# latticeboltzmann/2d-lb

Measured on AMD Instinct MI355X. Metric: MLUPS (million lattice updates per second), fused D2Q9 BGK step, higher is better.
Workload: dtype f32

## Files before the change

### 2d-lb_amd/csrc/kernels_deep.h

```cpp
#pragma once

#ifdef LB_DIAG
#define LB_DEEP_NOCOLLIDE if (!(a.diag & 1))
#else
#define LB_DEEP_NOCOLLIDE
#endif

namespace {

constexpr int DEEP_RW = 1, DEEP_PFD = 1;
constexpr int DEEP_WSLOTS = 8;
constexpr bool deep_pairs(bool mask, int bc) { return !mask && bc == LB_BC_PERIODIC; }

template <int RW, int NL>
struct DeepState {
    Window w[RW > 0 ? RW : 1];
    f4a d0[NL];
    unsigned mhist;
};
typedef unsigned u4v __attribute__((ext_vector_type(4)));
struct DeepCtx {
    int lane, x4, ym, n_iter;
    bool store_lane;
    f4a (*mine)[64], (*other)[64];
    f4a (*ho)[64];
    f4a (*dma)[64];
    unsigned dma_off;
};
constexpr int DEEP_WHOLE = 0, DEEP_FRONT = 1, DEEP_BACK = 2;
constexpr int DEEP_HO_SLOTS = 10;

__device__ __forceinline__ void deep_window_load(f4a (*W)[64], int lane, int it, f4a d0, Window &w)
{
    const int gs = 2 + 3 * (it & 1);
    w.d0 = d0; w.d1 = W[0][lane]; w.d3 = W[1][lane];
    w.g2 = W[gs][lane]; w.g5 = W[gs + 1][lane]; w.g6 = W[gs + 2][lane];
}
template <bool DOWN>
__device__ __forceinline__ void deep_window_push(f4a (*W)[64], int lane, int it, f4a &d0, const f4a (&q)[9])
{
    typedef Dir<DOWN> D_;
    const int gs = 2 + 3 * (it & 1);
    d0 = q[0]; W[0][lane] = q[1]; W[1][lane] = q[3];
    W[gs][lane] = q[D_::A]; W[gs + 1][lane] = q[D_::B]; W[gs + 2][lane] = q[D_::C];
}
template <bool DOWN>
__device__ __forceinline__ void deep_publish(f4a (*W)[64], int lane, int gs, const f4a (&q)[9])
{
    typedef Dir<DOWN> D_;
    W[gs][lane] = q[D_::An]; W[gs + 1][lane] = q[D_::Bn]; W[gs + 2][lane] = q[D_::Cn];
}

constexpr int DEEP_NUM_RECORDS = -1;
__device__ __forceinline__ float *deep_uniform(const float *p)
{
    const unsigned long long v = (unsigned long long)p;
    const unsigned lo = __builtin_amdgcn_readfirstlane((unsigned)v), hi = __builtin_amdgcn_readfirstlane((unsigned)(v >> 32));
    return reinterpret_cast<float *>(((unsigned long long)hi << 32) | lo);
}
__device__ __forceinline__ f4a deep_buf_load(__amdgpu_buffer_rsrc_t r, int vo, int so, int imm)
{
    return __builtin_bit_cast(f4a, __builtin_amdgcn_raw_buffer_load_b128(r, vo + imm, so, 0));
}
template <int BC, bool MASK>
__device__ __forceinline__ void deep_row_load(const StepArgs &a, int r, int x4, Row1 &o)
{
    int ym, yp;
    o.have = step1_rows(a, r, o.rr, ym, yp);
    o.mk = uc4{0, 0, 0, 0};
    o.hsolid = false;
    o.hxc = -1;
    if (o.have) {
        const long long P = a.pitch, S = a.plane;
        const float *s = a.src;
        const int yl = o.rr;
        o.wp = WrapPatch{0.f, 0.f, 0.f, 0.f, 0.f, 0.f};
        if (BC == LB_BC_PERIODIC) {
            const int c = a.nx - 1 - x4;
            const bool wrap_w = x4 == 0, wrap_e = c >= 0 && c < 4;
            if (wrap_w) {
                o.wp.p1 = s[1 * S + (long long)yl * P + a.nx - 1];
                o.wp.p5 = s[5 * S + (long long)ym * P + a.nx - 1];
                o.wp.p8 = s[8 * S + (long long)yp * P + a.nx - 1];
            }
            if (wrap_e) {
                o.wp.w3 = s[3 * S + (long long)yl * P];
                o.wp.w6 = s[6 * S + (long long)ym * P];
                o.wp.w7 = s[7 * S + (long long)yp * P];
            }
        }
        const __amdgpu_buffer_rsrc_t r0 = __builtin_amdgcn_make_buffer_rsrc(deep_uniform(s + (long long)yl * P - 1), 0, DEEP_NUM_RECORDS, 0x00020000);
        const __amdgpu_buffer_rsrc_t rm = __builtin_amdgcn_make_buffer_rsrc(deep_uniform(s + (long long)ym * P - 1), 0, DEEP_NUM_RECORDS, 0x00020000);
        const __amdgpu_buffer_rsrc_t rp = __builtin_amdgcn_make_buffer_rsrc(deep_uniform(s + (long long)yp * P - 1), 0, DEEP_NUM_RECORDS, 0x00020000);
        const unsigned S4 = (unsigned)a.plane * 4u;
        const int vo = x4 * 4;
        o.q[0] = deep_buf_load(r0, vo, 0, 4);
        o.q[1] = deep_buf_load(r0, vo, (int)(S4), 0);
        o.q[2] = deep_buf_load(rm, vo, (int)(2u * S4), 4);
        o.q[3] = deep_buf_load(r0, vo, (int)(3u * S4), 8);
        o.q[4] = deep_buf_load(rp, vo, (int)(4u * S4), 4);
        o.q[5] = deep_buf_load(rm, vo, (int)(5u * S4), 0);
        o.q[6] = deep_buf_load(rm, vo, (int)(6u * S4), 8);
        o.q[7] = deep_buf_load(rp, vo, (int)(7u * S4), 8);
        o.q[8] = deep_buf_load(rp, vo, (int)(8u * S4), 0);
        if (MASK) o.mk = *reinterpret_cast<const uc4 *>(lane_ptr(a.mask + (long long)yl * a.fpitch, x4));
    } else {
        o.wp = WrapPatch{0.f, 0.f, 0.f, 0.f, 0.f, 0.f};
#pragma unroll
        for (int k = 0; k < 9; ++k) o.q[k] = f4a{0.f, 0.f, 0.f, 0.f};
    }
}
#ifdef LB_DIAG
constexpr bool DEEP_MANUAL = false;
#else
constexpr bool DEEP_MANUAL = true;
#endif
__device__ __forceinline__ u4v deep_rsrc_words(const float *p)
{
    const unsigned long long v = (unsigned long long)p;
    return u4v{(unsigned)__builtin_amdgcn_readfirstlane((unsigned)v), (unsigned)__builtin_amdgcn_readfirstlane((unsigned)(v >> 32)), (unsigned)DEEP_NUM_RECORDS,
               0x00020000u};
}
template <int BC, bool MASK>
__device__ __forceinline__ void deep_row_issue(const StepArgs &a, int r, int x4, Row1 &o)
{
    int ym, yp;
    o.have = step1_rows(a, r, o.rr, ym, yp);
    o.hsolid = false;
    o.hxc = -1;
    if (o.have) {
        const long long P = a.pitch, S = a.plane;
        const float *s = a.src;
        const int yl = o.rr;
        if (BC == LB_BC_PERIODIC) {
            const int c = a.nx - 1 - x4;
            const bool wrap_w = x4 == 0, wrap_e = c >= 0 && c < 4;
            if (wrap_w) {
                const float *e = s + a.nx - 1;
                asm volatile("global_load_dword a36, %0, off\n\tglobal_load_dword a37, %1, off\n\tglobal_load_dword a38, %2, off"
                             :: "v"(e + 1 * S + (long long)yl * P), "v"(e + 5 * S + (long long)ym * P), "v"(e + 8 * S + (long long)yp * P)
                             : "memory", "a36", "a37", "a38");
            }
            if (wrap_e) {
                asm volatile("global_load_dword a39, %0, off\n\tglobal_load_dword a40, %1, off\n\tglobal_load_dword a41, %2, off"
                             :: "v"(s + 3 * S + (long long)yl * P), "v"(s + 6 * S + (long long)ym * P), "v"(s + 7 * S + (long long)yp * P)
                             : "memory", "a39", "a40", "a41");
            }
        }
        const u4v r0 = deep_rsrc_words(s + (long long)yl * P - 1), rm = deep_rsrc_words(s + (long long)ym * P - 1),
                  rp = deep_rsrc_words(s + (long long)yp * P - 1);
        const unsigned S4 = (unsigned)a.plane * 4u;
        asm volatile("buffer_load_dwordx4 a[0:3], %0, %1, 0 offen offset:4\n\t"
                     "buffer_load_dwordx4 a[4:7], %0, %1, %4 offen\n\t"
                     "buffer_load_dwordx4 a[8:11], %0, %2, %5 offen offset:4\n\t"
                     "buffer_load_dwordx4 a[12:15], %0, %1, %6 offen offset:8\n\t"
                     "buffer_load_dwordx4 a[16:19], %0, %3, %7 offen offset:4\n\t"
                     "buffer_load_dwordx4 a[20:23], %0, %2, %8 offen\n\t"
                     "buffer_load_dwordx4 a[24:27], %0, %2, %9 offen offset:8\n\t"
                     "buffer_load_dwordx4 a[28:31], %0, %3, %10 offen offset:8\n\t"
                     "buffer_load_dwordx4 a[32:35], %0, %3, %11 offen"
                     :: "v"(x4 * 4), "s"(r0), "s"(rm), "s"(rp), "s"(S4), "s"(2u * S4), "s"(3u * S4), "s"(4u * S4), "s"(5u * S4), "s"(6u * S4),
                        "s"(7u * S4), "s"(8u * S4)
                     : "memory", "a0", "a1", "a2", "a3", "a4", "a5", "a6", "a7", "a8", "a9", "a10", "a11", "a12", "a13",
                       "a14", "a15", "a16", "a17", "a18", "a19", "a20", "a21", "a22", "a23", "a24", "a25", "a26", "a27", "a28",
                       "a29", "a30", "a31", "a32", "a33", "a34", "a35");
        if (MASK) asm volatile("global_load_dword a42, %0, off" :: "v"(lane_ptr(a.mask + (long long)yl * a.fpitch, x4)) : "memory", "a42");
    }
}
template <int BC, bool MASK, int N>
__device__ __forceinline__ void deep_row_take(Row1 &o)
{
    static_assert(N == 0 || N == 9 || N == 12, "the stores of one steady iteration, or nothing");
#define LB_DEEP_TAKE_OUTS "={a[0:3]}"(o.q[0]), "={a[4:7]}"(o.q[1]), "={a[8:11]}"(o.q[2]), "={a[12:15]}"(o.q[3]), \
                          "={a[16:19]}"(o.q[4]), "={a[20:23]}"(o.q[5]), "={a[24:27]}"(o.q[6]), "={a[28:31]}"(o.q[7]), "={a[32:35]}"(o.q[8])
    if (N == 0) asm volatile("s_waitcnt vmcnt(0)" : LB_DEEP_TAKE_OUTS :: "memory");
    else if (N == 9) asm volatile("s_waitcnt vmcnt(9)" : LB_DEEP_TAKE_OUTS :: "memory");
    else asm volatile("s_waitcnt vmcnt(12)" : LB_DEEP_TAKE_OUTS :: "memory");
#undef LB_DEEP_TAKE_OUTS
    o.wp = WrapPatch{0.f, 0.f, 0.f, 0.f, 0.f, 0.f};
    if (BC == LB_BC_PERIODIC)
        asm volatile("" : "={a36}"(o.wp.p1), "={a37}"(o.wp.p5), "={a38}"(o.wp.p8), "={a39}"(o.wp.w3), "={a40}"(o.wp.w6), "={a41}"(o.wp.w7));
    o.mk = uc4{0, 0, 0, 0};
    if (MASK) {
        unsigned m;
        asm volatile("" : "={a42}"(m));
        o.mk = __builtin_bit_cast(uc4, m);
    }
    if (!o.have) {
#pragma unroll
        for (int k = 0; k < 9; ++k) o.q[k] = f4a{0.f, 0.f, 0.f, 0.f};
        o.mk = uc4{0, 0, 0, 0};
    }
}

template <int BC, bool MASK>
__device__ __forceinline__ void deep_row_issue_lds(const StepArgs &a, int r, int x4, unsigned slot, Row1 &o)
{
    int ym, yp;
    o.have = step1_rows(a, r, o.rr, ym, yp);
    o.hsolid = false;
    o.hxc = -1;
    if (o.have) {
        const long long P = a.pitch, S = a.plane;
        const float *s = a.src;
        const int yl = o.rr;
        unsigned m0_kept;
        asm volatile("s_waitcnt lgkmcnt(0)" ::: "memory");
        if (BC == LB_BC_PERIODIC) {
            const int c = a.nx - 1 - x4;
            const bool wrap_w = x4 == 0, wrap_e = c >= 0 && c < 4;
            if (wrap_w) {
                const float *e = s + a.nx - 1;
                asm volatile("s_mov_b32 %0, m0\n\ts_mov_b32 m0, %4\n\ts_nop 0\n\tglobal_load_lds_dword %1, off\n\t"
                             "s_add_u32 m0, m0, 0x100\n\ts_nop 0\n\tglobal_load_lds_dword %2, off\n\t"
                             "s_add_u32 m0, m0, 0x100\n\ts_nop 0\n\tglobal_load_lds_dword %3, off\n\ts_mov_b32 m0, %0"
                             : "=&s"(m0_kept)
                             : "v"(e + 1 * S + (long long)yl * P), "v"(e + 5 * S + (long long)ym * P), "v"(e + 8 * S + (long long)yp * P),
                               "s"(slot + 9 * 1024 + 256)
                             : "memory", "scc");
            }
            if (wrap_e) {
                asm volatile("s_mov_b32 %0, m0\n\ts_mov_b32 m0, %4\n\ts_nop 0\n\tglobal_load_lds_dword %1, off\n\t"
                             "s_add_u32 m0, m0, 0x100\n\ts_nop 0\n\tglobal_load_lds_dword %2, off\n\t"
                             "s_add_u32 m0, m0, 0x100\n\ts_nop 0\n\tglobal_load_lds_dword %3, off\n\ts_mov_b32 m0, %0"
                             : "=&s"(m0_kept)
                             : "v"(s + 3 * S + (long long)yl * P), "v"(s + 6 * S + (long long)ym * P), "v"(s + 7 * S + (long long)yp * P),
                               "s"(slot + 9 * 1024 + 256)
                             : "memory", "scc");
            }
        }
        const u4v r0 = deep_rsrc_words(s + (long long)yl * P - 1), rm = deep_rsrc_words(s + (long long)ym * P - 1),
                  rp = deep_rsrc_words(s + (long long)yp * P - 1);
        const unsigned S4 = (unsigned)a.plane * 4u;
        const int v0 = x4 * 4, v4 = v0 + 4, v8 = v0 + 8;
        asm volatile("s_mov_b32 %0, m0\n\ts_mov_b32 m0, %15\n\ts_nop 0\n\tbuffer_load_dwordx4 %2, %4, 0 offen lds\n\t"
                     "s_add_u32 m0, m0, 0x400\n\ts_nop 0\n\tbuffer_load_dwordx4 %1, %4, %7 offen lds\n\t"
                     "s_add_u32 m0, m0, 0x400\n\ts_nop 0\n\tbuffer_load_dwordx4 %2, %5, %8 offen lds\n\t"
                     "s_add_u32 m0, m0, 0x400\n\ts_nop 0\n\tbuffer_load_dwordx4 %3, %4, %9 offen lds\n\t"
                     "s_add_u32 m0, m0, 0x400\n\ts_nop 0\n\tbuffer_load_dwordx4 %2, %6, %10 offen lds\n\t"
                     "s_add_u32 m0, m0, 0x400\n\ts_nop 0\n\tbuffer_load_dwordx4 %1, %5, %11 offen lds\n\t"
                     "s_add_u32 m0, m0, 0x400\n\ts_nop 0\n\tbuffer_load_dwordx4 %3, %5, %12 offen lds\n\t"
                     "s_add_u32 m0, m0, 0x400\n\ts_nop 0\n\tbuffer_load_dwordx4 %3, %6, %13 offen lds\n\t"
                     "s_add_u32 m0, m0, 0x400\n\ts_nop 0\n\tbuffer_load_dwordx4 %1, %6, %14 offen lds\n\ts_mov_b32 m0, %0"
                     : "=&s"(m0_kept)
                     : "v"(v0), "v"(v4), "v"(v8), "s"(r0), "s"(rm), "s"(rp), "s"(S4), "s"(2u * S4), "s"(3u * S4), "s"(4u * S4), "s"(5u * S4),
                       "s"(6u * S4), "s"(7u * S4), "s"(8u * S4), "s"(slot)
                     : "memory", "scc");
        if (MASK)
            asm volatile("s_mov_b32 %0, m0\n\ts_mov_b32 m0, %2\n\ts_nop 0\n\tglobal_load_lds_dword %1, off\n\ts_mov_b32 m0, %0"
                         : "=&s"(m0_kept) : "v"(lane_ptr(a.mask + (long long)yl * a.fpitch, x4)), "s"(slot + 9 * 1024) : "memory");
    }
}
template <int BC, bool MASK>
__device__ __forceinline__ void deep_row_take_lds(const f4a (*S)[64], int lane, Row1 &o)
{
    asm volatile("s_waitcnt vmcnt(0)" ::: "memory");
    if (o.have) {
#pragma unroll
        for (int k = 0; k < 9; ++k) o.q[k] = S[k][lane];
        const unsigned *X = reinterpret_cast<const unsigned *>(S[9]);
        o.mk = MASK ? __builtin_bit_cast(uc4, X[lane]) : uc4{0, 0, 0, 0};
        o.wp = WrapPatch{0.f, 0.f, 0.f, 0.f, 0.f, 0.f};
        if (BC == LB_BC_PERIODIC) {
            const float e1 = __builtin_bit_cast(float, X[64 + lane]), e2 = __builtin_bit_cast(float, X[128 + lane]),
                        e3 = __builtin_bit_cast(float, X[192 + lane]);
            o.wp = WrapPatch{e1, e2, e3, e1, e2, e3};
        }
    } else {
        o.wp = WrapPatch{0.f, 0.f, 0.f, 0.f, 0.f, 0.f};
#pragma unroll
        for (int k = 0; k < 9; ++k) o.q[k] = f4a{0.f, 0.f, 0.f, 0.f};
        o.mk = uc4{0, 0, 0, 0};
    }
}

__device__ __forceinline__ void deep_row_store(const StepArgs &a, int r, int x4, const f4a (&t)[9])
{
    const __amdgpu_buffer_rsrc_t rd = __builtin_amdgcn_make_buffer_rsrc(deep_uniform(a.dst + (long long)r * a.pitch), 0, DEEP_NUM_RECORDS, 0x00020000);
    const unsigned S4 = (unsigned)a.plane * 4u;
    const int vo = x4 * 4;
    asm volatile("" ::: "memory");
    if (a.nts != 0) {
#pragma unroll
        for (int k = 0; k < 9; ++k) __builtin_amdgcn_raw_buffer_store_b128(__builtin_bit_cast(u4v, t[k]), rd, vo, (int)(k * S4), 2);
    } else {
#pragma unroll
        for (int k = 0; k < 9; ++k) __builtin_amdgcn_raw_buffer_store_b128(__builtin_bit_cast(u4v, t[k]), rd, vo, (int)(k * S4), 0);
    }
}

template <int BC, bool MASK, bool MACRO, int D, int RW, bool DOWN, int NST, int S, int ROLE = DEEP_WHOLE>
__device__ __forceinline__ void deep_stage(const StepArgs &a, const DeepCtx &cx, const int i, const int it,
                                           DeepState<RW, D - 1 - RW> &st, f4a (&qin)[9], f4a &r4, f4a &u4, f4a &v4)
{
    if constexpr (S <= D) {
        constexpr int K = S - 1;
        const int lane = cx.lane, x4 = cx.x4;
        constexpr int L = K > RW ? K - RW - 1 : 0;
        f4a (*W)[64] = cx.mine + L * DEEP_WSLOTS;
        if constexpr (NST >= S) {
            int r, t0_, t1_;
            (void)step1_rows(a, DOWN ? cx.ym - 1 - (i - K) : cx.ym + (i - K), r, t0_, t1_);
            f4a t[9];
            if constexpr (K <= RW) {
                skirt_gather<DOWN>(st.w[K - 1], qin, t);
                window_push_dir<DOWN>(st.w[K - 1], qin);
            } else {
                Window w;
                deep_window_load(W, lane, it, st.d0[L], w);
                skirt_gather<DOWN>(w, qin, t);
                deep_window_push<DOWN>(W, lane, it, st.d0[L], qin);
            }
            LB_DEEP_NOCOLLIDE collide_row<BC, MASK, true>(a, x4, a.y0 + r, t, mask_bits(st.mhist, K), r4, u4, v4);
            if constexpr (S == D && ROLE == DEEP_FRONT) {
#pragma unroll
                for (int k = 0; k < 9; ++k) cx.ho[k][lane] = t[k];
                if (MASK) reinterpret_cast<unsigned *>(cx.ho[9])[lane] = __builtin_bit_cast(unsigned, mask_bits(st.mhist, K));
            } else if constexpr (S == D) {
#ifdef LB_DIAG
                if (!(a.diag & (1 << 22)))
#endif
                if (cx.store_lane) {
                    deep_row_store(a, r, x4, t);
                    if (MACRO) {
                        const long long m = (long long)r * a.fpitch;
                        store_moments(a, m, x4, r4, u4, v4);
                    }
                }
            } else {
                if constexpr (NST == S) {
                    if constexpr (S <= RW) deep_publish<DOWN>(cx.other + (D - 2 - RW) * DEEP_WSLOTS, lane, S == 1 ? 5 : 2, t);
                    else deep_publish<DOWN>(cx.other + (S - RW - 1) * DEEP_WSLOTS, lane, 2 + 3 * (S & 1), t);
                }
                deep_stage<BC, MASK, MACRO, D, RW, DOWN, NST, S + 1, ROLE>(a, cx, i, it, st, t, r4, u4, v4);
            }
        } else if constexpr (NST == S - 1) {
            if constexpr (K <= RW) window_push_dir<DOWN>(st.w[K - 1], qin);
            else deep_window_push<DOWN>(W, lane, it, st.d0[L], qin);
        }
    }
}

template <int BC, bool MASK, bool MACRO, int D, int RW, int PFD, bool DOWN, int NST, int PAR = -1, int ROLE = DEEP_WHOLE>
__device__ __forceinline__ void deep_iter(const StepArgs &a, const DeepCtx &cx, const int i_, DeepState<RW, D - 1 - RW> &st, Row1 &cur,
                                          Row1 &nxt)
{
    static_assert(RW >= 0 && RW <= 2 && D - 1 - RW >= 1 && (ROLE == DEEP_WHOLE ? D - 2 > RW : D - 2 >= RW),
                  "register windows hand over through the last LDS window while it is idle");
    static_assert((D - 1 - RW) * DEEP_WSLOTS <= 40, "a wave has 40 KB of LDS at four waves per CU");
    const int lane = cx.lane, x4 = cx.x4;
    const int i = NST < D ? NST - 1 : i_;
    const int it = PAR >= 0 ? PAR : i;
    auto row_at = [&](int p) { return DOWN ? cx.ym - 1 - p : cx.ym + p; };
    f4a (*MB)[64] = cx.mine + (D - 2 - RW) * DEEP_WSLOTS;
    if (RW >= 1 && NST == 2) { st.w[0].g2 = MB[5][lane]; st.w[0].g5 = MB[6][lane]; st.w[0].g6 = MB[7][lane]; }
    if (RW >= 2 && NST == 3) { st.w[RW >= 2 ? 1 : 0].g2 = MB[2][lane]; st.w[RW >= 2 ? 1 : 0].g5 = MB[3][lane]; st.w[RW >= 2 ? 1 : 0].g6 = MB[4][lane]; }
#ifdef LB_DIAG
    if (!((a.diag & (1 << 23)) && i > 0))
#endif
    if constexpr (ROLE != DEEP_BACK) {
        if (ROLE == DEEP_FRONT) {
            deep_row_take_lds<BC, MASK>(cx.dma, lane, cur);
            deep_row_issue_lds<BC, MASK>(a, row_at(min(i + 1, cx.n_iter - 1)), x4, cx.dma_off, nxt);
        } else if (PFD && DEEP_MANUAL) {
            deep_row_take<BC, MASK, (NST < D ? 0 : (MACRO ? 12 : 9))>(cur);
            deep_row_issue<BC, MASK>(a, row_at(min(i + 1, cx.n_iter - 1)), x4, nxt);
        } else {
            static_assert(PFD == 1 || ROLE == DEEP_BACK, "a march that gathers its rows gathers them one ahead");
            deep_row_load<BC, MASK>(a, row_at(min(i + 1, cx.n_iter - 1)), x4, nxt);
        }
    }
    f4a (&q1)[9] = cur.q;
    f4a r4, u4, v4;
    const uc4 mk = cur.mk;
    if (ROLE != DEEP_BACK && cur.have) {
        gather_merge<BC, true>(a, x4, q1, cur.wp);
        LB_DEEP_NOCOLLIDE collide_row<BC, MASK, true>(a, x4, a.y0 + cur.rr, q1, mk, r4, u4, v4);
    }
    if (NST == 1) {
        if constexpr (RW >= 1) deep_publish<DOWN>(cx.other + (D - 2 - RW) * DEEP_WSLOTS, lane, 5, q1);
        else deep_publish<DOWN>(cx.other, lane, 2 + 3 * 1, q1);
    }
    deep_stage<BC, MASK, MACRO, D, RW, DOWN, NST, 2, ROLE>(a, cx, i, it, st, q1, r4, u4, v4);
    if (MASK) st.mhist = ((st.mhist | mask_word(mk)) << 1) & (0x01010101u * (unsigned)(((1 << D) - 2) & 0xff));
    if (ROLE == DEEP_WHOLE && NST < D) __syncthreads();
}

template <int BC, bool MASK, bool MACRO, int D, int RW, int PFD, bool DOWN, int NST>
__device__ __forceinline__ void deep_fill(const StepArgs &a, const DeepCtx &cx, DeepState<RW, D - 1 - RW> &st, Row1 &ra, Row1 &rb)
{
    if constexpr (NST < D) {
        if ((NST & 1) == 0) deep_iter<BC, MASK, MACRO, D, RW, PFD, DOWN, NST>(a, cx, NST - 1, st, rb, ra);
        else deep_iter<BC, MASK, MACRO, D, RW, PFD, DOWN, NST>(a, cx, NST - 1, st, ra, rb);
        deep_fill<BC, MASK, MACRO, D, RW, PFD, DOWN, NST + 1>(a, cx, st, ra, rb);
    }
}

template <int BC, bool MASK, bool MACRO, int D, int RW, int PFD, bool DOWN>
__device__ __forceinline__ void deep_march(const StepArgs &a, const int x0, const int ym, const int len, f4a (*mine)[64],
                                           f4a (*other)[64])
{
    DeepCtx cx;
    cx.lane = threadIdx.x;
    const int xr = x0 + cx.lane * 4;
    cx.x4 = skirt_column<BC>(a, xr, deep_skirt_lanes(D));
    cx.store_lane = skirt_store_lane(a, cx.lane, xr, deep_skirt_lanes(D));
    cx.ym = ym; cx.n_iter = len + D - 1;
    cx.mine = mine; cx.other = other;
    DeepState<RW, D - 1 - RW> st = {};
    auto row_at = [&](int p) { return DOWN ? ym - 1 - p : ym + p; };
    static_assert(PFD == 1, "a whole march gathers one row ahead");
    Row1 ra, rb;
    if (DEEP_MANUAL) deep_row_issue<BC, MASK>(a, row_at(0), cx.x4, ra);
    else deep_row_load<BC, MASK>(a, row_at(0), cx.x4, ra);
    deep_fill<BC, MASK, MACRO, D, RW, PFD, DOWN, 1>(a, cx, st, ra, rb);
    if (DEEP_MANUAL) asm volatile("s_waitcnt vmcnt(0)" ::: "memory");
    if (!deep_pairs(MASK, BC)) {
        if ((D - 1) & 1) ra = rb;
        for (int i = D - 1; i < cx.n_iter; ++i) {
            deep_iter<BC, MASK, MACRO, D, RW, PFD, DOWN, D>(a, cx, i, st, ra, rb);
            ra = rb;
        }
    } else {
        constexpr int P0 = (D - 1) & 1;
        int i = D - 1;
        for (; i + 1 < cx.n_iter; i += 2) {
            deep_iter<BC, MASK, MACRO, D, RW, PFD, DOWN, D, P0>(a, cx, i, st, P0 ? rb : ra, P0 ? ra : rb);
            deep_iter<BC, MASK, MACRO, D, RW, PFD, DOWN, D, 1 - P0>(a, cx, i + 1, st, P0 ? ra : rb, P0 ? rb : ra);
        }
        if (i < cx.n_iter) deep_iter<BC, MASK, MACRO, D, RW, PFD, DOWN, D, P0>(a, cx, i, st, P0 ? rb : ra, P0 ? ra : rb);
    }
    if (DEEP_MANUAL) asm volatile("s_waitcnt vmcnt(0)" ::: "memory");
}

template <int BC, bool MASK, bool MACRO, int D, int RW, int PFD>
__global__ __launch_bounds__(64 * STEP4_WAVES, PFD ? 1 : 2) void k_deep(const StepArgs a, int strips, int seg_rows, int nsegs, int row_end)
{
    __shared__ f4a lds_win[STEP4_WAVES][(D - 1 - RW) * DEEP_WSLOTS][64];
    const int wy = __builtin_amdgcn_readfirstlane(threadIdx.y);
    const int item = xcd_item(blockIdx.x, gridDim.x);
#ifdef LB_DIAG
    const unsigned long long diag_t0 = __builtin_amdgcn_s_memrealtime();
#endif
    int sx, sy;
    if (item < strips * nsegs) {
        sx = item % strips;
        sy = item / strips;
    } else {
        if (!a.edge_seg_rows) return;
        const int j = item - strips * nsegs;
        sx = (j & 1) ? strips - 1 : 0;
        sy = nsegs + (j >> 1);
    }
    int stride = a.seg_stride;
    if (a.edge_seg_rows && (sx == 0 || sx == strips - 1)) stride = seg_rows = a.edge_seg_rows;
    const int ya = a.row_begin + sy * stride;
    if (ya >= row_end) return;
    const int yb = min(ya + seg_rows, row_end);
    const int ym = ya + (yb - ya) / 2;
    const int x0 = sx * deep_valid(D) - 4 * deep_skirt_lanes(D);
    if (wy == 0) deep_march<BC, MASK, MACRO, D, RW, PFD, true>(a, x0, ym, ym - ya, lds_win[0], lds_win[1]);
    else deep_march<BC, MASK, MACRO, D, RW, PFD, false>(a, x0, ym, yb - ym, lds_win[1], lds_win[0]);
#ifdef LB_DIAG
    if ((a.diag & 4096) && threadIdx.x == 0) {
        __builtin_amdgcn_s_waitcnt(0);
        const unsigned long long t1 = __builtin_amdgcn_s_memrealtime();
        unsigned *o = reinterpret_cast<unsigned *>(a.rho) + 8 * (item * STEP4_WAVES + wy);
// ... 10 lines not shown
```

### 2d-lb_amd/csrc/kernels_deep2.h

```cpp
#pragma once

namespace {

constexpr int deep2_split(int D) { return D >= 8 ? 4 : (D + 1) / 2; }
constexpr int deep2_rw_front(int D) { return deep2_split(D) - 2 >= 2 ? 2 : 1; }
constexpr int deep2_rw_back(int D) { return (D - deep2_split(D) + 1) - 2 >= 2 ? 2 : 1; }
constexpr int DEEP2_WAVES = 4;

__device__ __forceinline__ void deep2_barrier() { asm volatile("s_waitcnt lgkmcnt(0)\n\ts_barrier" ::: "memory"); }

template <int BC, bool MASK, int F, int RW, bool DOWN, int NST>
__device__ __forceinline__ void deep2_front_fill(const StepArgs &a, const DeepCtx &cx, DeepState<RW, F - 1 - RW> &st, Row1 &ra, Row1 &rb,
                                                 int &trip)
{
    if constexpr (NST < F) {
        deep2_barrier();
        if (trip < cx.n_iter) {
            if ((NST & 1) == 0) deep_iter<BC, MASK, false, F, RW, 1, DOWN, NST, -1, DEEP_FRONT>(a, cx, NST - 1, st, rb, ra);
            else deep_iter<BC, MASK, false, F, RW, 1, DOWN, NST, -1, DEEP_FRONT>(a, cx, NST - 1, st, ra, rb);
        }
        deep2_barrier();
        ++trip;
        deep2_front_fill<BC, MASK, F, RW, DOWN, NST + 1>(a, cx, st, ra, rb, trip);
    }
}

template <int BC, bool MASK, int D, int F, int RW, bool DOWN>
__device__ __forceinline__ void deep2_front(const StepArgs &a, const int x0, const int ym, const int len, const int trips, f4a (*mine)[64],
                                            f4a (*other)[64], f4a (*ho)[64], f4a (*dma)[64])
{
    DeepCtx cx;
    cx.lane = threadIdx.x;
    const int xr = x0 + cx.lane * 4;
    cx.x4 = skirt_column<BC>(a, xr, deep_skirt_lanes(D));
    cx.store_lane = false;
    cx.ym = ym; cx.n_iter = len + D - 1;
    cx.mine = mine; cx.other = other; cx.ho = ho; cx.dma = dma;
    cx.dma_off = __builtin_amdgcn_readfirstlane((unsigned)reinterpret_cast<unsigned long long>(dma));
    DeepState<RW, F - 1 - RW> st = {};
    auto row_at = [&](int p) { return DOWN ? ym - 1 - p : ym + p; };
    Row1 ra, rb;
    deep_row_issue_lds<BC, MASK>(a, row_at(0), cx.x4, cx.dma_off, ra);
    int trip = 0;
    deep2_front_fill<BC, MASK, F, RW, DOWN, 1>(a, cx, st, ra, rb, trip);
    if ((F - 1) & 1) ra = rb;
    for (; trip < trips; ++trip) {
#ifdef LB_DIAG
        if (!(a.diag & (1 << 24)))
#endif
        deep2_barrier();
        if (trip < cx.n_iter) {
            deep_iter<BC, MASK, false, F, RW, 1, DOWN, F, -1, DEEP_FRONT>(a, cx, trip, st, ra, rb);
            ra = rb;
        }
#ifdef LB_DIAG
        if (!(a.diag & (1 << 24)))
#endif
        deep2_barrier();
    }
    asm volatile("s_waitcnt vmcnt(0)" ::: "memory");
}

template <bool MASK>
__device__ __forceinline__ void deep2_take(const DeepCtx &cx, Row1 &cur)
{
#pragma unroll
    for (int k = 0; k < 9; ++k) cur.q[k] = cx.ho[k][cx.lane];
    cur.mk = uc4{0, 0, 0, 0};
    if (MASK) cur.mk = __builtin_bit_cast(uc4, reinterpret_cast<const unsigned *>(cx.ho[9])[cx.lane]);
    cur.have = true;
}

template <int BC, bool MASK, bool MACRO, int DB, int RW, bool DOWN, int NST>
__device__ __forceinline__ void deep2_back_fill(const StepArgs &a, const DeepCtx &cx, DeepState<RW, DB - 1 - RW> &st, Row1 &cur, int &j)
{
    if constexpr (NST < DB) {
        if (j < cx.n_iter) deep2_take<MASK>(cx, cur);
        deep2_barrier();
        if (j < cx.n_iter) deep_iter<BC, MASK, MACRO, DB, RW, 0, DOWN, NST, -1, DEEP_BACK>(a, cx, NST - 1, st, cur, cur);
        deep2_barrier();
        ++j;
        deep2_back_fill<BC, MASK, MACRO, DB, RW, DOWN, NST + 1>(a, cx, st, cur, j);
    }
}

template <int BC, bool MASK, bool MACRO, int D, int F, int RW, bool DOWN>
__device__ __forceinline__ void deep2_back(const StepArgs &a, const int x0, const int ym, const int len, const int trips, f4a (*mine)[64],
                                           f4a (*other)[64], f4a (*ho)[64])
{
    constexpr int DB = D - F + 1;
    DeepCtx cx;
    cx.lane = threadIdx.x;
    const int xr = x0 + cx.lane * 4;
    cx.x4 = skirt_column<BC>(a, xr, deep_skirt_lanes(D));
    cx.store_lane = skirt_store_lane(a, cx.lane, xr, deep_skirt_lanes(D));
    cx.ym = ym; cx.n_iter = len + DB - 1;
    cx.mine = mine; cx.other = other; cx.ho = ho;
    DeepState<RW, DB - 1 - RW> st = {};
    Row1 cur;
    cur.wp = WrapPatch{0.f, 0.f, 0.f, 0.f, 0.f, 0.f};
    cur.hsolid = false; cur.hxc = -1; cur.rr = 0;
    for (int t = 0; t < F; ++t) {
        deep2_barrier();
        deep2_barrier();
    }
    int j = 0;
    deep2_back_fill<BC, MASK, MACRO, DB, RW, DOWN, 1>(a, cx, st, cur, j);
    for (; j + F < trips; ++j) {
        if (j < cx.n_iter) deep2_take<MASK>(cx, cur);
#ifdef LB_DIAG
        if (!(a.diag & (1 << 24)))
#endif
        deep2_barrier();
        if (j < cx.n_iter) deep_iter<BC, MASK, MACRO, DB, RW, 0, DOWN, DB, -1, DEEP_BACK>(a, cx, j, st, cur, cur);
#ifdef LB_DIAG
        if (!(a.diag & (1 << 24)))
#endif
        deep2_barrier();
    }
}

template <int BC, bool MASK, bool MACRO, int D>
__global__ __launch_bounds__(64 * DEEP2_WAVES, 2) void k_deep2(const StepArgs a, int strips, int seg_rows, int nsegs, int row_end)
{
    constexpr int F = deep2_split(D), RWF = deep2_rw_front(D), RWB = deep2_rw_back(D);
    constexpr int LF = (F - 1 - RWF) * DEEP_WSLOTS, LBK = (D - F - RWB) * DEEP_WSLOTS;
    static_assert(2 * (LF + LBK + 2 * DEEP_HO_SLOTS) <= 80, "two workgroups per CU: 80 KB each");
    __shared__ f4a lds_dma[2][DEEP_HO_SLOTS][64];
    __shared__ f4a lds_front[2][LF][64];
    __shared__ f4a lds_back[2][LBK][64];
    __shared__ f4a lds_ho[2][DEEP_HO_SLOTS][64];
    const int wy = (__builtin_amdgcn_readfirstlane(threadIdx.y) + ((blockIdx.x >> 8) & 1) * 2) & 3;
    const int item = xcd_item(blockIdx.x, gridDim.x);
#ifdef LB_DIAG
    const unsigned long long diag_t0 = __builtin_amdgcn_s_memrealtime();
#endif
    int sx, sy;
    if (item < strips * nsegs) {
        sx = item % strips;
        sy = item / strips;
    } else {
        if (!a.edge_seg_rows) return;
        const int j = item - strips * nsegs;
        sx = (j & 1) ? strips - 1 : 0;
        sy = nsegs + (j >> 1);
    }
    int stride = a.seg_stride;
    if (a.edge_seg_rows && (sx == 0 || sx == strips - 1)) stride = seg_rows = a.edge_seg_rows;
    const int ya = a.row_begin + sy * stride;
    if (ya >= row_end) return;
    const int yb = min(ya + seg_rows, row_end);
// ... 22 lines not shown
```

### 2d-lb_amd/csrc/kernels_step5.h

```cpp
#pragma once

namespace {


struct March5State {
    Window w1, w2;
    unsigned mhist;
};
struct March5Ctx {
    int lane, x4, ym, n_iter, wy;
    bool store_lane;
    unsigned slot;
    f4a (*W3)[64], (*W4)[64], (*P3)[64], (*P4)[64];
    f4a (*R2)[64], (*Q2)[64];
};

__device__ __forceinline__ float wave_from_left(float v)
{
    const int i = __builtin_bit_cast(int, v);
    return __builtin_bit_cast(float, __builtin_amdgcn_update_dpp(0, i, 0x138, 0xf, 0xf, true));
}
__device__ __forceinline__ float wave_from_right(float v)
{
    const int i = __builtin_bit_cast(int, v);
    return __builtin_bit_cast(float, __builtin_amdgcn_update_dpp(0, i, 0x130, 0xf, 0xf, true));
}
__device__ __forceinline__ f4a skirt_left(f4a v) { return f4a{wave_from_left(v.w), v.x, v.y, v.z}; }
__device__ __forceinline__ f4a skirt_right(f4a v) { return f4a{v.y, v.z, v.w, wave_from_right(v.x)}; }
template <bool DOWN>
__device__ __forceinline__ void skirt_gather(const Window &w, const f4a (&q)[9], f4a (&t)[9])
{
    typedef Dir<DOWN> D;
    t[0] = w.d0;
    t[1] = skirt_left(w.d1);
    t[3] = skirt_right(w.d3);
    t[D::A] = w.g2;
    t[D::B] = skirt_left(w.g5);
    t[D::C] = skirt_right(w.g6);
    t[D::An] = q[D::An];
    t[D::Cn] = skirt_right(q[D::Cn]);
    t[D::Bn] = skirt_left(q[D::Bn]);
}

template <int BC, bool MASK, bool MACRO, bool PF, bool DOWN, int NST>
__device__ __forceinline__ void march5_iter(const StepArgs &a, const March5Ctx &cx, const int i_, March5State &st, Row1 &cur)
{
    const int lane = cx.lane, x4 = cx.x4;
    const long long S = a.plane;
    const int i = NST < 5 ? NST - 1 : i_;
    const int it = i;
    auto row_at = [&](int p) { return DOWN ? cx.ym - 1 - p : cx.ym + p; };
    f4a(*W3)[64] = cx.W3;
    f4a(*W4)[64] = cx.W4;
    Window &w1 = st.w1, &w2 = st.w2;

    prio_turn(a, i, cx.slot);
    if (NST == 2) { w1.g2 = W4[6][lane]; w1.g5 = W4[7][lane]; w1.g6 = W4[8][lane]; }
    if (NST == 3 && !PF) { w2.g2 = W4[3][lane]; w2.g5 = W4[4][lane]; w2.g6 = W4[5][lane]; }
    if (!PF) row1_load<BC, MASK>(a, row_at(i), x4, false, 0, cur);
    f4a (&q1)[9] = cur.q;
    f4a r4, u4, v4;
    const uc4 mk = cur.mk;
    if (cur.have) {
        gather_merge<BC, true>(a, x4, q1, cur.wp);
        collide_row<BC, MASK>(a, x4, a.y0 + cur.rr, q1, mk, r4, u4, v4);
    }
    const int r_next = row_at(min(i + 1, cx.n_iter - 1));
    if (NST == 1) lds_publish<DOWN>(cx.P4, lane, 6, q1);
    f4a q2[9];
    if (NST >= 2) {
        int r2, t0_, t1_;
        (void)step1_rows(a, row_at(i - 1), r2, t0_, t1_);
        skirt_gather<DOWN>(w1, q1, q2);
        window_push_dir<DOWN>(w1, q1);
        if (PF) row1_load<BC, MASK>(a, r_next, x4, false, 0, cur);
        collide_row<BC, MASK>(a, x4, a.y0 + r2, q2, mask_bits(st.mhist, 1), r4, u4, v4);
        if (NST == 2) {
            if (PF) lds_publish<DOWN>(cx.Q2, lane, 0, q2);
            else lds_publish<DOWN>(cx.P4, lane, 3, q2);
        }
    } else {
// ... 131 lines not shown
```

Baseline: 474,500.

## Carry running row base pointers through deep march instead of recomputing addresses

Replaces the per-iteration row index computation (step1_rows, 64-bit pitch multiplies, readfirstlane of addresses) with a DeepRows struct holding running source, destination and mask row bases that are advanced incrementally, with explicit wrap handling for periodic y. It also rewrites the skirt lane shifts to use a packed v_pk_mov_b32 for the middle pair. The aim is to cut scalar/vector address arithmetic in the inner march loop. This adds more live state and subtle wrap logic; the velocity-inlet case is statically excluded.

```diff
diff --git a/2d-lb_amd/csrc/kernels_deep.h b/2d-lb_amd/csrc/kernels_deep.h
--- a/2d-lb_amd/csrc/kernels_deep.h
+++ b/2d-lb_amd/csrc/kernels_deep.h
@@ -19,7 +19,17 @@
     unsigned mhist;
 };
 typedef unsigned u4v __attribute__((ext_vector_type(4)));
+struct DeepRows {
+    unsigned long long b0, bm, bp;
+    unsigned long long bd;
+    unsigned long long m0;
+    int rr;
+    int ri;
+    unsigned long long bq_wrap, mq, mq_wrap;
+    int yq;
+};
 struct DeepCtx {
+    DeepRows rows;
     int lane, x4, ym, n_iter;
     bool store_lane;
     f4a (*mine)[64], (*other)[64];
@@ -52,46 +62,113 @@
 }
 
 constexpr int DEEP_NUM_RECORDS = -1;
-__device__ __forceinline__ float *deep_uniform(const float *p)
-{
-    const unsigned long long v = (unsigned long long)p;
-    const unsigned lo = __builtin_amdgcn_readfirstlane((unsigned)v), hi = __builtin_amdgcn_readfirstlane((unsigned)(v >> 32));
-    return reinterpret_cast<float *>(((unsigned long long)hi << 32) | lo);
-}
 __device__ __forceinline__ f4a deep_buf_load(__amdgpu_buffer_rsrc_t r, int vo, int so, int imm)
 {
     return __builtin_bit_cast(f4a, __builtin_amdgcn_raw_buffer_load_b128(r, vo + imm, so, 0));
 }
+template <int BC>
+__device__ __forceinline__ bool deep_wraps(const StepArgs &a)
+{
+    static_assert(BC != LB_BC_VELOCITY_INLET, "the running row bases know wrap_y 0 and 1");
+    return BC == LB_BC_PERIODIC && a.wrap_y != 0;
+}
+template <int BC>
+__device__ __forceinline__ int deep_wrap_row(const StepArgs &a, int r)
+{
+    const int wr = r < 0 ? r + a.h : (r >= a.h ? r - a.h : r);
+    return deep_wraps<BC>(a) ? wr : r;
+}
+template <int BC>
+__device__ __forceinline__ bool deep_rows_have(const StepArgs &a, const DeepRows &w)
+{
+    return deep_wraps<BC>(a) || (w.rr < 0 ? a.ghost_s != 0 : (w.rr >= a.h ? a.ghost_n != 0 : true));
+}
+template <int BC, bool MASK, bool DOWN>
+__device__ __forceinline__ void deep_rows_init(const StepArgs &a, int ym_line, int depth, DeepRows &w)
+{
+    const unsigned long long s = (unsigned long long)a.src, P4 = (unsigned long long)((long long)a.pitch * 4);
+    const int r0 = DOWN ? ym_line - 1 : ym_line;
+    int ym, yp;
+    (void)step1_rows(a, r0, w.rr, ym, yp);
+    w.b0 = s + (unsigned long long)w.rr * P4;
+    w.bm = s + (unsigned long long)ym * P4;
+    w.bp = s + (unsigned long long)yp * P4;
+    w.yq = DOWN ? ym : yp;
+    w.bq_wrap = DOWN ? s + (unsigned long long)(a.h - 1) * P4 : s;
+    w.ri = r0;
+    w.bd = (unsigned long long)a.dst + (unsigned long long)(DOWN ? r0 + (depth - 1) : r0 - (depth - 1)) * P4;
+    w.m0 = w.mq = w.mq_wrap = 0;
+    if (MASK) {
+        const unsigned long long m = (unsigned long long)a.mask, F = (unsigned long long)(long long)a.fpitch;
+        w.m0 = m + (unsigned long long)w.rr * F;
+        w.mq = m + (unsigned long long)w.yq * F;
+        w.mq_wrap = DOWN ? m + (unsigned long long)(a.h - 1) * F : m;
+    }
+}
+template <int BC, bool MASK, bool DOWN>
+__device__ __forceinline__ void deep_rows_step(const StepArgs &a, DeepRows &w)
+{
+    constexpr int dir = DOWN ? -1 : 1;
+    const unsigned long long P4 = (unsigned long long)((long long)a.pitch * (4 * dir)), F = (unsigned long long)(long long)(DOWN ? -a.fpitch : a.fpitch);
+    if constexpr (BC == LB_BC_PERIODIC) {
+        unsigned long long &lead = DOWN ? w.bm : w.bp, &trail = DOWN ? w.bp : w.bm;
+        const int y1 = w.yq + dir;
+        const bool wrap = deep_wraps<BC>(a) && (DOWN ? y1 < 0 : y1 >= a.h);
+        trail = w.b0;
+        w.b0 = lead;
+        lead = wrap ? w.bq_wrap : lead + P4;
+        w.rr = w.yq;
+        w.yq = wrap ? (DOWN ? a.h - 1 : 0) : y1;
+        if (MASK) {
+            w.m0 = w.mq;
+            w.mq = wrap ? w.mq_wrap : w.mq + F;
+        }
+    } else {
+        const unsigned long long Pup = (unsigned long long)((long long)a.pitch * 4);
+        w.b0 += P4;
+        w.bm = w.b0 - Pup;
+        w.bp = w.b0 + Pup;
+        if (MASK) w.m0 += F;
+        w.rr += dir;
+    }
+}
+template <bool DOWN>
+__device__ __forceinline__ void deep_rows_next(const StepArgs &a, DeepRows &w)
+{
+    w.ri += DOWN ? -1 : 1;
+    w.bd += (unsigned long long)((long long)a.pitch * (DOWN ? -4 : 4));
+}
+__device__ __forceinline__ const float *deep_row_ptr(unsigned long long b) { return reinterpret_cast<const float *>(b); }
+
 template <int BC, bool MASK>
-__device__ __forceinline__ void deep_row_load(const StepArgs &a, int r, int x4, Row1 &o)
-{
-    int ym, yp;
-    o.have = step1_rows(a, r, o.rr, ym, yp);
+__device__ __forceinline__ void deep_row_load(const StepArgs &a, const DeepRows &w, int x4, Row1 &o)
+{
+    o.have = deep_rows_have<BC>(a, w);
+    o.rr = w.rr;
     o.mk = uc4{0, 0, 0, 0};
     o.hsolid = false;
     o.hxc = -1;
     if (o.have) {
-        const long long P = a.pitch, S = a.plane;
-        const float *s = a.src;
-        const int yl = o.rr;
+        const long long S = a.plane;
+        const float *s0 = deep_row_ptr(w.b0), *sm = deep_row_ptr(w.bm), *sp = deep_row_ptr(w.bp);
         o.wp = WrapPatch{0.f, 0.f, 0.f, 0.f, 0.f, 0.f};
         if (BC == LB_BC_PERIODIC) {
             const int c = a.nx - 1 - x4;
             const bool wrap_w = x4 == 0, wrap_e = c >= 0 && c < 4;
             if (wrap_w) {
-                o.wp.p1 = s[1 * S + (long long)yl * P + a.nx - 1];
-                o.wp.p5 = s[5 * S + (long long)ym * P + a.nx - 1];
-                o.wp.p8 = s[8 * S + (long long)yp * P + a.nx - 1];
+                o.wp.p1 = s0[1 * S + a.nx - 1];
+                o.wp.p5 = sm[5 * S + a.nx - 1];
+                o.wp.p8 = sp[8 * S + a.nx - 1];
             }
             if (wrap_e) {
-                o.wp.w3 = s[3 * S + (long long)yl * P];
-                o.wp.w6 = s[6 * S + (long long)ym * P];
-                o.wp.w7 = s[7 * S + (long long)yp * P];
-            }
-        }
-        const __amdgpu_buffer_rsrc_t r0 = __builtin_amdgcn_make_buffer_rsrc(deep_uniform(s + (long long)yl * P - 1), 0, DEEP_NUM_RECORDS, 0x00020000);
-        const __amdgpu_buffer_rsrc_t rm = __builtin_amdgcn_make_buffer_rsrc(deep_uniform(s + (long long)ym * P - 1), 0, DEEP_NUM_RECORDS, 0x00020000);
-        const __amdgpu_buffer_rsrc_t rp = __builtin_amdgcn_make_buffer_rsrc(deep_uniform(s + (long long)yp * P - 1), 0, DEEP_NUM_RECORDS, 0x00020000);
+                o.wp.w3 = s0[3 * S];
+                o.wp.w6 = sm[6 * S];
+                o.wp.w7 = sp[7 * S];
+            }
+        }
+        const __amdgpu_buffer_rsrc_t r0 = __builtin_amdgcn_make_buffer_rsrc(const_cast<float *>(s0 - 1), 0, DEEP_NUM_RECORDS, 0x00020000);
+        const __amdgpu_buffer_rsrc_t rm = __builtin_amdgcn_make_buffer_rsrc(const_cast<float *>(sm - 1), 0, DEEP_NUM_RECORDS, 0x00020000);
+        const __amdgpu_buffer_rsrc_t rp = __builtin_amdgcn_make_buffer_rsrc(const_cast<float *>(sp - 1), 0, DEEP_NUM_RECORDS, 0x00020000);
         const unsigned S4 = (unsigned)a.plane * 4u;
         const int vo = x4 * 4;
         o.q[0] = deep_buf_load(r0, vo, 0, 4);
@@ -103,7 +180,7 @@
         o.q[6] = deep_buf_load(rm, vo, (int)(6u * S4), 8);
         o.q[7] = deep_buf_load(rp, vo, (int)(7u * S4), 8);
         o.q[8] = deep_buf_load(rp, vo, (int)(8u * S4), 0);
-        if (MASK) o.mk = *reinterpret_cast<const uc4 *>(lane_ptr(a.mask + (long long)yl * a.fpitch, x4));
+        if (MASK) o.mk = *reinterpret_cast<const uc4 *>(lane_ptr(reinterpret_cast<const uint8_t *>(w.m0), x4));
     } else {
         o.wp = WrapPatch{0.f, 0.f, 0.f, 0.f, 0.f, 0.f};
 #pragma unroll
@@ -115,40 +192,37 @@
 #else
 constexpr bool DEEP_MANUAL = true;
 #endif
-__device__ __forceinline__ u4v deep_rsrc_words(const float *p)
-{
-    const unsigned long long v = (unsigned long long)p;
-    return u4v{(unsigned)__builtin_amdgcn_readfirstlane((unsigned)v), (unsigned)__builtin_amdgcn_readfirstlane((unsigned)(v >> 32)), (unsigned)DEEP_NUM_RECORDS,
-               0x00020000u};
+__device__ __forceinline__ u4v deep_rsrc_words(unsigned long long b)
+{
+    const unsigned long long v = b - 4;
+    return u4v{(unsigned)v, (unsigned)(v >> 32), (unsigned)DEEP_NUM_RECORDS, 0x00020000u};
 }
 template <int BC, bool MASK>
-__device__ __forceinline__ void deep_row_issue(const StepArgs &a, int r, int x4, Row1 &o)
-{
-    int ym, yp;
-    o.have = step1_rows(a, r, o.rr, ym, yp);
+__device__ __forceinline__ void deep_row_issue(const StepArgs &a, const DeepRows &w, int x4, Row1 &o)
+{
+    o.have = deep_rows_have<BC>(a, w);
+    o.rr = w.rr;
     o.hsolid = false;
     o.hxc = -1;
     if (o.have) {
-        const long long P = a.pitch, S = a.plane;
-        const float *s = a.src;
-        const int yl = o.rr;
+        const long long S = a.plane;
+        const float *s0 = deep_row_ptr(w.b0), *sm = deep_row_ptr(w.bm), *sp = deep_row_ptr(w.bp);
         if (BC == LB_BC_PERIODIC) {
             const int c = a.nx - 1 - x4;
             const bool wrap_w = x4 == 0, wrap_e = c >= 0 && c < 4;
             if (wrap_w) {
-                const float *e = s + a.nx - 1;
+                const long long e = a.nx - 1;
                 asm volatile("global_load_dword a36, %0, off\n\tglobal_load_dword a37, %1, off\n\tglobal_load_dword a38, %2, off"
-                             :: "v"(e + 1 * S + (long long)yl * P), "v"(e + 5 * S + (long long)ym * P), "v"(e + 8 * S + (long long)yp * P)
+                             :: "v"(s0 + (1 * S + e)), "v"(sm + (5 * S + e)), "v"(sp + (8 * S + e))
                              : "memory", "a36", "a37", "a38");
             }
             if (wrap_e) {
                 asm volatile("global_load_dword a39, %0, off\n\tglobal_load_dword a40, %1, off\n\tglobal_load_dword a41, %2, off"
-                             :: "v"(s + 3 * S + (long long)yl * P), "v"(s + 6 * S + (long long)ym * P), "v"(s + 7 * S + (long long)yp * P)
+                             :: "v"(s0 + 3 * S), "v"(sm + 6 * S), "v"(sp + 7 * S)
                              : "memory", "a39", "a40", "a41");
             }
         }
-        const u4v r0 = deep_rsrc_words(s + (long long)yl * P - 1), rm = deep_rsrc_words(s + (long long)ym * P - 1),
-                  rp = deep_rsrc_words(s + (long long)yp * P - 1);
+        const u4v r0 = deep_rsrc_words(w.b0), rm = deep_rsrc_words(w.bm), rp = deep_rsrc_words(w.bp);
         const unsigned S4 = (unsigned)a.plane * 4u;
         asm volatile("buffer_load_dwordx4 a[0:3], %0, %1, 0 offen offset:4\n\t"
                      "buffer_load_dwordx4 a[4:7], %0, %1, %4 offen\n\t"
@@ -164,7 +238,7 @@
                      : "memory", "a0", "a1", "a2", "a3", "a4", "a5", "a6", "a7", "a8", "a9", "a10", "a11", "a12", "a13",
                        "a14", "a15", "a16", "a17", "a18", "a19", "a20", "a21", "a22", "a23", "a24", "a25", "a26", "a27", "a28",
                        "a29", "a30", "a31", "a32", "a33", "a34", "a35");
-        if (MASK) asm volatile("global_load_dword a42, %0, off" :: "v"(lane_ptr(a.mask + (long long)yl * a.fpitch, x4)) : "memory", "a42");
+        if (MASK) asm volatile("global_load_dword a42, %0, off" :: "v"(lane_ptr(reinterpret_cast<const uint8_t *>(w.m0), x4)) : "memory", "a42");
     }
 }
 template <int BC, bool MASK, int N>
@@ -194,29 +268,27 @@
 }
 
 template <int BC, bool MASK>
-__device__ __forceinline__ void deep_row_issue_lds(const StepArgs &a, int r, int x4, unsigned slot, Row1 &o)
-{
-    int ym, yp;
-    o.have = step1_rows(a, r, o.rr, ym, yp);
+__device__ __forceinline__ void deep_row_issue_lds(const StepArgs &a, const DeepRows &w, int x4, unsigned slot, Row1 &o)
+{
+    o.have = deep_rows_have<BC>(a, w);
+    o.rr = w.rr;
     o.hsolid = false;
     o.hxc = -1;
     if (o.have) {
-        const long long P = a.pitch, S = a.plane;
-        const float *s = a.src;
-        const int yl = o.rr;
+        const long long S = a.plane;
+        const float *s0 = deep_row_ptr(w.b0), *sm = deep_row_ptr(w.bm), *sp = deep_row_ptr(w.bp);
         unsigned m0_kept;
         asm volatile("s_waitcnt lgkmcnt(0)" ::: "memory");
         if (BC == LB_BC_PERIODIC) {
             const int c = a.nx - 1 - x4;
             const bool wrap_w = x4 == 0, wrap_e = c >= 0 && c < 4;
             if (wrap_w) {
-                const float *e = s + a.nx - 1;
+                const long long e = a.nx - 1;
                 asm volatile("s_mov_b32 %0, m0\n\ts_mov_b32 m0, %4\n\ts_nop 0\n\tglobal_load_lds_dword %1, off\n\t"
                              "s_add_u32 m0, m0, 0x100\n\ts_nop 0\n\tglobal_load_lds_dword %2, off\n\t"
                              "s_add_u32 m0, m0, 0x100\n\ts_nop 0\n\tglobal_load_lds_dword %3, off\n\ts_mov_b32 m0, %0"
                              : "=&s"(m0_kept)
-                             : "v"(e + 1 * S + (long long)yl * P), "v"(e + 5 * S + (long long)ym * P), "v"(e + 8 * S + (long long)yp * P),
-                               "s"(slot + 9 * 1024 + 256)
+                             : "v"(s0 + (1 * S + e)), "v"(sm + (5 * S + e)), "v"(sp + (8 * S + e)), "s"(slot + 9 * 1024 + 256)
                              : "memory", "scc");
             }
             if (wrap_e) {
@@ -224,13 +296,11 @@
                              "s_add_u32 m0, m0, 0x100\n\ts_nop 0\n\tglobal_load_lds_dword %2, off\n\t"
                              "s_add_u32 m0, m0, 0x100\n\ts_nop 0\n\tglobal_load_lds_dword %3, off\n\ts_mov_b32 m0, %0"
                              : "=&s"(m0_kept)
-                             : "v"(s + 3 * S + (long long)yl * P), "v"(s + 6 * S + (long long)ym * P), "v"(s + 7 * S + (long long)yp * P),
-                               "s"(slot + 9 * 1024 + 256)
+                             : "v"(s0 + 3 * S), "v"(sm + 6 * S), "v"(sp + 7 * S), "s"(slot + 9 * 1024 + 256)
                              : "memory", "scc");
             }
         }
-        const u4v r0 = deep_rsrc_words(s + (long long)yl * P - 1), rm = deep_rsrc_words(s + (long long)ym * P - 1),
-                  rp = deep_rsrc_words(s + (long long)yp * P - 1);
+        const u4v r0 = deep_rsrc_words(w.b0), rm = deep_rsrc_words(w.bm), rp = deep_rsrc_words(w.bp);
         const unsigned S4 = (unsigned)a.plane * 4u;
         const int v0 = x4 * 4, v4 = v0 + 4, v8 = v0 + 8;
         asm volatile("s_mov_b32 %0, m0\n\ts_mov_b32 m0, %15\n\ts_nop 0\n\tbuffer_load_dwordx4 %2, %4, 0 offen lds\n\t"
@@ -248,7 +318,7 @@
                      : "memory", "scc");
         if (MASK)
             asm volatile("s_mov_b32 %0, m0\n\ts_mov_b32 m0, %2\n\ts_nop 0\n\tglobal_load_lds_dword %1, off\n\ts_mov_b32 m0, %0"
-                         : "=&s"(m0_kept) : "v"(lane_ptr(a.mask + (long long)yl * a.fpitch, x4)), "s"(slot + 9 * 1024) : "memory");
+                         : "=&s"(m0_kept) : "v"(lane_ptr(reinterpret_cast<const uint8_t *>(w.m0), x4)), "s"(slot + 9 * 1024) : "memory");
     }
 }
 template <int BC, bool MASK>
@@ -274,9 +344,9 @@
     }
 }
 
-__device__ __forceinline__ void deep_row_store(const StepArgs &a, int r, int x4, const f4a (&t)[9])
-{
-    const __amdgpu_buffer_rsrc_t rd = __builtin_amdgcn_make_buffer_rsrc(deep_uniform(a.dst + (long long)r * a.pitch), 0, DEEP_NUM_RECORDS, 0x00020000);
+__device__ __forceinline__ void deep_row_store(const StepArgs &a, const DeepRows &w, int x4, const f4a (&t)[9])
+{
+    const __amdgpu_buffer_rsrc_t rd = __builtin_amdgcn_make_buffer_rsrc(reinterpret_cast<float *>(w.bd), 0, DEEP_NUM_RECORDS, 0x00020000);
     const unsigned S4 = (unsigned)a.plane * 4u;
     const int vo = x4 * 4;
     asm volatile("" ::: "memory");
@@ -299,8 +369,7 @@
         constexpr int L = K > RW ? K - RW - 1 : 0;
         f4a (*W)[64] = cx.mine + L * DEEP_WSLOTS;
         if constexpr (NST >= S) {
-            int r, t0_, t1_;
-            (void)step1_rows(a, DOWN ? cx.ym - 1 - (i - K) : cx.ym + (i - K), r, t0_, t1_);
+            const int r = deep_wrap_row<BC>(a, DOWN ? cx.rows.ri + K : cx.rows.ri - K);
             f4a t[9];
             if constexpr (K <= RW) {
                 skirt_gather<DOWN>(st.w[K - 1], qin, t);
@@ -321,7 +390,7 @@
                 if (!(a.diag & (1 << 22)))
 #endif
                 if (cx.store_lane) {
-                    deep_row_store(a, r, x4, t);
+                    deep_row_store(a, cx.rows, x4, t);
                     if (MACRO) {
                         const long long m = (long long)r * a.fpitch;
                         store_moments(a, m, x4, r4, u4, v4);
@@ -342,7 +411,7 @@
 }
 
 template <int BC, bool MASK, bool MACRO, int D, int RW, int PFD, bool DOWN, int NST, int PAR = -1, int ROLE = DEEP_WHOLE>
-__device__ __forceinline__ void deep_iter(const StepArgs &a, const DeepCtx &cx, const int i_, DeepState<RW, D - 1 - RW> &st, Row1 &cur,
+__device__ __forceinline__ void deep_iter(const StepArgs &a, DeepCtx &cx, const int i_, DeepState<RW, D - 1 - RW> &st, Row1 &cur,
                                           Row1 &nxt)
 {
     static_assert(RW >= 0 && RW <= 2 && D - 1 - RW >= 1 && (ROLE == DEEP_WHOLE ? D - 2 > RW : D - 2 >= RW),
@@ -351,7 +420,6 @@
     const int lane = cx.lane, x4 = cx.x4;
     const int i = NST < D ? NST - 1 : i_;
     const int it = PAR >= 0 ? PAR : i;
-    auto row_at = [&](int p) { return DOWN ? cx.ym - 1 - p : cx.ym + p; };
     f4a (*MB)[64] = cx.mine + (D - 2 - RW) * DEEP_WSLOTS;
     if (RW >= 1 && NST == 2) { st.w[0].g2 = MB[5][lane]; st.w[0].g5 = MB[6][lane]; st.w[0].g6 = MB[7][lane]; }
     if (RW >= 2 && NST == 3) { st.w[RW >= 2 ? 1 : 0].g2 = MB[2][lane]; st.w[RW >= 2 ? 1 : 0].g5 = MB[3][lane]; st.w[RW >= 2 ? 1 : 0].g6 = MB[4][lane]; }
@@ -359,15 +427,16 @@
     if (!((a.diag & (1 << 23)) && i > 0))
 #endif
     if constexpr (ROLE != DEEP_BACK) {
+        if (i + 1 < cx.n_iter) deep_rows_step<BC, MASK, DOWN>(a, cx.rows);
         if (ROLE == DEEP_FRONT) {
             deep_row_take_lds<BC, MASK>(cx.dma, lane, cur);
-            deep_row_issue_lds<BC, MASK>(a, row_at(min(i + 1, cx.n_iter - 1)), x4, cx.dma_off, nxt);
+            deep_row_issue_lds<BC, MASK>(a, cx.rows, x4, cx.dma_off, nxt);
         } else if (PFD && DEEP_MANUAL) {
             deep_row_take<BC, MASK, (NST < D ? 0 : (MACRO ? 12 : 9))>(cur);
-            deep_row_issue<BC, MASK>(a, row_at(min(i + 1, cx.n_iter - 1)), x4, nxt);
+            deep_row_issue<BC, MASK>(a, cx.rows, x4, nxt);
         } else {
             static_assert(PFD == 1 || ROLE == DEEP_BACK, "a march that gathers its rows gathers them one ahead");
-            deep_row_load<BC, MASK>(a, row_at(min(i + 1, cx.n_iter - 1)), x4, nxt);
+            deep_row_load<BC, MASK>(a, cx.rows, x4, nxt);
         }
     }
     f4a (&q1)[9] = cur.q;
@@ -383,11 +452,12 @@
     }
     deep_stage<BC, MASK, MACRO, D, RW, DOWN, NST, 2, ROLE>(a, cx, i, it, st, q1, r4, u4, v4);
     if (MASK) st.mhist = ((st.mhist | mask_word(mk)) << 1) & (0x01010101u * (unsigned)(((1 << D) - 2) & 0xff));
+    deep_rows_next<DOWN>(a, cx.rows);
     if (ROLE == DEEP_WHOLE && NST < D) __syncthreads();
 }
 
 template <int BC, bool MASK, bool MACRO, int D, int RW, int PFD, bool DOWN, int NST>
-__device__ __forceinline__ void deep_fill(const StepArgs &a, const DeepCtx &cx, DeepState<RW, D - 1 - RW> &st, Row1 &ra, Row1 &rb)
+__device__ __forceinline__ void deep_fill(const StepArgs &a, DeepCtx &cx, DeepState<RW, D - 1 - RW> &st, Row1 &ra, Row1 &rb)
 {
     if constexpr (NST < D) {
         if ((NST & 1) == 0) deep_iter<BC, MASK, MACRO, D, RW, PFD, DOWN, NST>(a, cx, NST - 1, st, rb, ra);
@@ -408,11 +478,11 @@
     cx.ym = ym; cx.n_iter = len + D - 1;
     cx.mine = mine; cx.other = other;
     DeepState<RW, D - 1 - RW> st = {};
-    auto row_at = [&](int p) { return DOWN ? ym - 1 - p : ym + p; };
     static_assert(PFD == 1, "a whole march gathers one row ahead");
+    deep_rows_init<BC, MASK, DOWN>(a, ym, D, cx.rows);
     Row1 ra, rb;
-    if (DEEP_MANUAL) deep_row_issue<BC, MASK>(a, row_at(0), cx.x4, ra);
-    else deep_row_load<BC, MASK>(a, row_at(0), cx.x4, ra);
+    if (DEEP_MANUAL) deep_row_issue<BC, MASK>(a, cx.rows, cx.x4, ra);
+    else deep_row_load<BC, MASK>(a, cx.rows, cx.x4, ra);
     deep_fill<BC, MASK, MACRO, D, RW, PFD, DOWN, 1>(a, cx, st, ra, rb);
     if (DEEP_MANUAL) asm volatile("s_waitcnt vmcnt(0)" ::: "memory");
     if (!deep_pairs(MASK, BC)) {
diff --git a/2d-lb_amd/csrc/kernels_deep2.h b/2d-lb_amd/csrc/kernels_deep2.h
--- a/2d-lb_amd/csrc/kernels_deep2.h
+++ b/2d-lb_amd/csrc/kernels_deep2.h
@@ -10,7 +10,7 @@
 __device__ __forceinline__ void deep2_barrier() { asm volatile("s_waitcnt lgkmcnt(0)\n\ts_barrier" ::: "memory"); }
 
 template <int BC, bool MASK, int F, int RW, bool DOWN, int NST>
-__device__ __forceinline__ void deep2_front_fill(const StepArgs &a, const DeepCtx &cx, DeepState<RW, F - 1 - RW> &st, Row1 &ra, Row1 &rb,
+__device__ __forceinline__ void deep2_front_fill(const StepArgs &a, DeepCtx &cx, DeepState<RW, F - 1 - RW> &st, Row1 &ra, Row1 &rb,
                                                  int &trip)
 {
     if constexpr (NST < F) {
@@ -38,9 +38,9 @@
     cx.mine = mine; cx.other = other; cx.ho = ho; cx.dma = dma;
     cx.dma_off = __builtin_amdgcn_readfirstlane((unsigned)reinterpret_cast<unsigned long long>(dma));
     DeepState<RW, F - 1 - RW> st = {};
-    auto row_at = [&](int p) { return DOWN ? ym - 1 - p : ym + p; };
+    deep_rows_init<BC, MASK, DOWN>(a, ym, F, cx.rows);
     Row1 ra, rb;
-    deep_row_issue_lds<BC, MASK>(a, row_at(0), cx.x4, cx.dma_off, ra);
+    deep_row_issue_lds<BC, MASK>(a, cx.rows, cx.x4, cx.dma_off, ra);
     int trip = 0;
     deep2_front_fill<BC, MASK, F, RW, DOWN, 1>(a, cx, st, ra, rb, trip);
     if ((F - 1) & 1) ra = rb;
@@ -72,7 +72,7 @@
 }
 
 template <int BC, bool MASK, bool MACRO, int DB, int RW, bool DOWN, int NST>
-__device__ __forceinline__ void deep2_back_fill(const StepArgs &a, const DeepCtx &cx, DeepState<RW, DB - 1 - RW> &st, Row1 &cur, int &j)
+__device__ __forceinline__ void deep2_back_fill(const StepArgs &a, DeepCtx &cx, DeepState<RW, DB - 1 - RW> &st, Row1 &cur, int &j)
 {
     if constexpr (NST < DB) {
         if (j < cx.n_iter) deep2_take<MASK>(cx, cur);
@@ -97,6 +97,7 @@
     cx.ym = ym; cx.n_iter = len + DB - 1;
     cx.mine = mine; cx.other = other; cx.ho = ho;
     DeepState<RW, DB - 1 - RW> st = {};
+    deep_rows_init<BC, MASK, DOWN>(a, ym, DB, cx.rows);
     Row1 cur;
     cur.wp = WrapPatch{0.f, 0.f, 0.f, 0.f, 0.f, 0.f};
     cur.hsolid = false; cur.hxc = -1; cur.rr = 0;
diff --git a/2d-lb_amd/csrc/kernels_step5.h b/2d-lb_amd/csrc/kernels_step5.h
--- a/2d-lb_amd/csrc/kernels_step5.h
+++ b/2d-lb_amd/csrc/kernels_step5.h
@@ -25,8 +25,23 @@
     const int i = __builtin_bit_cast(int, v);
     return __builtin_bit_cast(float, __builtin_amdgcn_update_dpp(0, i, 0x130, 0xf, 0xf, true));
 }
-__device__ __forceinline__ f4a skirt_left(f4a v) { return f4a{wave_from_left(v.w), v.x, v.y, v.z}; }
-__device__ __forceinline__ f4a skirt_right(f4a v) { return f4a{v.y, v.z, v.w, wave_from_right(v.x)}; }
+typedef float f2a __attribute__((ext_vector_type(2)));
+__device__ __forceinline__ f2a skirt_straddle(f4a v)
+{
+    f2a r;
+    asm("v_pk_mov_b32 %0, %1, %2 op_sel:[1,0]" : "=v"(r) : "v"(__builtin_shufflevector(v, v, 0, 1)), "v"(__builtin_shufflevector(v, v, 2, 3)));
+    return r;
+}
+__device__ __forceinline__ f4a skirt_left(f4a v)
+{
+    const f2a m = skirt_straddle(v);
+    return f4a{wave_from_left(v.w), v.x, m.x, m.y};
+}
+__device__ __forceinline__ f4a skirt_right(f4a v)
+{
+    const f2a m = skirt_straddle(v);
+    return f4a{m.x, m.y, v.w, wave_from_right(v.x)};
+}
 template <bool DOWN>
 __device__ __forceinline__ void skirt_gather(const Window &w, const f4a (&q)[9], f4a (&t)[9])
 {
```

After: 482,900, median of 6. About the same (+1.8%).
